# calderpg/fast_kinematic_simulator

Hardware: NVIDIA B200
Metric: particle-microsteps/sec (with contact resolution) (higher is better)
Workload: dtype f64

## Files before the change

### fast_kinematic_simulator_b200/csrc/fks_api.cu

```cuda

#include <cuda_runtime.h>
#include <nvtx3/nvToolsExt.h>

#include <algorithm>
#include <cmath>
#include <cstdio>
#include <cstdlib>
#include <cstring>
#include <new>
#include <string>
#include <vector>

#include "fks_device_types.h"
#include "fks_internal.h"

using namespace fksdev;

namespace fks_host {
static thread_local std::string g_last_error;
void set_last_error(const std::string& msg) { g_last_error = msg; }

void finish_env_l2_window(fks_env* env) {
    cudaDeviceProp prop;
    if (cudaGetDeviceProperties(&prop, env->device) == cudaSuccess && prop.persistingL2CacheMaxSize > 0) {
// ... 521 lines not shown
    s->last_stream = nullptr;
    s->has_last = false;
    {
        int lim = 0;
        if (cudaDeviceGetAttribute(&lim, cudaDevAttrMaxSharedMemoryPerBlockOptin, env->device) != cudaSuccess || lim <= 0) lim = 48 * 1024;
        s->smem_limit = (size_t)lim;
    }
    s->launches = 0;
    s->d_trace = nullptr;
    s->d_trace_count = nullptr;
    s->trace_capacity = 0;
    const double freq = std::fabs(simulation_controller_frequency);
    s->sp.interval = 1.0 / simulation_controller_frequency;
    s->sp.shortcut_distance = params->simulation_shortcut_distance;
    s->sp.check_tolerance = params->environment_collision_check_tolerance;
    s->sp.decay_rate = params->resolve_correction_step_scaling_decay_rate;
    s->sp.initial_step = params->resolve_correction_initial_step_size;
    s->sp.min_scaling = params->resolve_correction_min_step_scaling;
    s->sp.max_iters = params->max_resolver_iterations;
    s->sp.decay_iters = params->resolve_correction_step_scaling_decay_iterations;
    s->sp.n_steps = std::max((uint32_t)(params->forward_simulation_time * freq), 1u);
    s->sp.failed_ends_motion = params->failed_resolves_end_motion ? 1 : 0;

    const DevRobot& h = robot->host;
    std::memset(&s->plan, 0, sizeof(s->plan));
    int wpb = kWarpsPerBlock;
    if (const char* ev = std::getenv("FKS_WARPS_PER_BLOCK")) {
        const int v = std::atoi(ev);
        if (v >= 1 && v <= kWarpsPerBlock) wpb = v;
    }
    int rc = 0;
    for (;; wpb = (wpb > 4) ? wpb - 4 : wpb - 1) {
        s->dyn_smem = simulate_smem_plan(&s->plan, h.L, h.J, h.D, h.P, robot->stride, wpb, s->smem_limit);
        s->kinfo.max_blocks_per_sm = 0;
        rc = simulate_kernel_info(h.kind, s->dyn_smem, wpb, &s->kinfo);
        if ((rc == 0 && s->kinfo.max_blocks_per_sm >= 1) || wpb <= 1) break;
        cudaGetLastError();
    }
    s->plan.cull_mode = 1;
    s->plan.trace = nullptr;
    s->plan.trace_count = nullptr;
    s->plan.trace_capacity = 0;
    s->plan.trace_width = 0;
    if (const char* ev = std::getenv("FKS_CULL")) s->plan.cull_mode = std::atoi(ev);
    if (rc != 0) { delete s; return cuda_fail((cudaError_t)rc, "fks_sim_create: kernel attributes"); }
    if (s->kinfo.max_blocks_per_sm < 1) { delete s; return fail(FKS_ERR_UNSUPPORTED, "fks_sim_create: robot does not fit one CTA's shared memory"); }
    cudaDeviceProp prop;
    cudaError_t err = cudaGetDeviceProperties(&prop, s->device);
    if (err != cudaSuccess) { delete s; return cuda_fail(err, "cudaGetDeviceProperties"); }
    s->grid_max = prop.multiProcessorCount * s->kinfo.max_blocks_per_sm;
    s->num_sms = prop.multiProcessorCount;
    s->pool_eighths = 16;
    if (const char* ev = std::getenv("FKS_POOL_EIGHTHS")) s->pool_eighths = std::max(8, std::atoi(ev));
    s->pool = std::min((s->pool_eighths * wpb + 7) / 8, kMaxPool);
    const size_t scratch_bytes = (size_t)s->grid_max * s->pool * s->plan.sl.total;
    const size_t jscratch_bytes = (size_t)s->grid_max * wpb * s->plan.sl.jtotal;
    s->plan.pool = s->pool;
    s->plan.ctx_stride = (int)context_bytes(s->plan.wl);
    const size_t ctx_bytes = (size_t)s->grid_max * s->pool * (size_t)s->plan.ctx_stride;

    if ((err = cudaStreamCreateWithFlags(&s->stream, cudaStreamNonBlocking)) != cudaSuccess ||
        (err = cudaEventCreateWithFlags(&s->last_done, cudaEventDisableTiming)) != cudaSuccess ||
        (err = cudaMalloc((void**)&s->d_scratch, scratch_bytes)) != cudaSuccess ||
        (err = cudaMalloc((void**)&s->d_jscratch, jscratch_bytes)) != cudaSuccess ||
        (err = cudaMalloc((void**)&s->d_ctx_store, ctx_bytes)) != cudaSuccess ||
        (err = cudaMalloc((void**)&s->d_stats, 128 * sizeof(unsigned long long))) != cudaSuccess ||
        (err = cudaMalloc((void**)&s->d_counter, 4 * sizeof(unsigned int))) != cudaSuccess ||
        (err = cudaMemset(s->d_stats, 0, 128 * sizeof(unsigned long long))) != cudaSuccess) {
        fks_sim_destroy(s);
        return cuda_fail(err, "fks_sim_create: allocation");
    }
    char buf[512];
    std::snprintf(buf, sizeof(buf),
                  "simulate_kernel<kind=%d>: %d regs/thread, %zu B dynamic smem/CTA, %d B local/thread, %d threads/CTA, "
                  "%d CTAs/SM x %d SMs (persistent grid %d), scratch %llu B/warp, L2 window %zu B",
                  h.kind, s->kinfo.regs, s->dyn_smem, s->kinfo.local_bytes, 32 * wpb, s->kinfo.max_blocks_per_sm,
                  prop.multiProcessorCount, s->grid_max, (unsigned long long)s->plan.sl.jtotal, env->l2_window_bytes);
// ... 630 lines not shown
```

### fast_kinematic_simulator_b200/csrc/fks_device_types.h

```cpp
#ifndef FKS_DEVICE_TYPES_H
#define FKS_DEVICE_TYPES_H

#include <stdint.h>

#include "fksgpu.h"

namespace fksdev {

constexpr int kMaxDof = 16;
constexpr int kMaxLinks = 16;
constexpr int kMaxJoints = 16;
constexpr int kMaxPairs = (kMaxLinks * (kMaxLinks - 1)) / 2;
constexpr int kMaxSelfPartners = kMaxLinks - 1;
constexpr int kPairChunks = (kMaxPairs + 31) / 32;
#ifndef FKS_MAX_WARPS
#define FKS_MAX_WARPS 24
#endif
constexpr int kWarpsPerBlock = FKS_MAX_WARPS;
constexpr int kThreadsPerBlock = kWarpsPerBlock * 32;

struct DevAxis {
    double kp, ki, kd, iclamp;
    double vlim;
    double pnoise, mnoise;
// ... 81 lines not shown
    int M;
    int jsm;
    int jsm_ld;
    int jsm_big_ld;
    int jaxis, jorig;
    int target, scfg, act, ru, du, raw, stepv;
    int tn;
    int qr;
    int cand;
    int vars;
    int flags;
    int save2_end;
    int stats;
    int total;
    int noise_batch;
};

inline __host__ __device__ WarpLayout make_warp_layout(int L, int J, int D, int stride, int jsm_extra = 0) {
    WarpLayout w;
    int S = stride > D ? stride : D;
    S = (S + 1) & ~1;
    w.S = S;
    w.L12 = 12 * L;
    w.noise_batch = 32 / D < 1 ? 1 : (32 / D > 8 ? 8 : 32 / D);
    int o = 0;
    w.cfg = o; o += 3 * S;
    w.T = o; o += 3 * w.L12;
    w.jsm = w.T + 2 * w.L12;
    w.M = o; o += 16 * J;
    w.caps = o; o += 6 * L;
    o += jsm_extra;
    auto pick_ld = [](int doubles, int columns) {
        const int cap = doubles / columns;
        int ld = cap;
        const int pref = cap - ((cap - 4) & 15);
        if (cap >= 20 && pref >= 20 && pref * 4 >= cap * 3) ld = pref;
        return ld < 0 ? 0 : ld;
    };
    w.jsm_ld = pick_ld(o - w.jsm, D + 1);
    o += (14 + 16 - (o - w.T) % 16) % 16;
    w.G = o; o += w.L12;
    w.jaxis = o; o += 3 * J;
    w.jorig = o; o += 3 * J;
    o = (o + 1) & ~1;
    w.cand = o; o += 32;
    w.jsm_big_ld = pick_ld(o - w.jsm, D + 1);
    w.target = o; o += S;
    w.scfg = o; o += S;
    w.act = o; o += S;
    w.ru = o; o += S;
    w.du = o; o += S;
    w.raw = o; o += S;
    w.stepv = o; o += S;
    w.tn = o; o += w.noise_batch * S;
    w.vars = o; o += kWarpVarsDoubles + 2 * S;
    w.flags = o; o += 1;
    w.save2_end = o;
    w.qr = o; o += S;
    w.stats = o; o += FKS_NUM_STATS;
    w.total = (o + 1) & ~1;
    return w;
}

struct ScratchLayout {
    unsigned long long selfcorr;
    unsigned long long selfwork;
    unsigned long long keys;
// ... 52 lines not shown
    int pool, ctx_stride;
    unsigned long long n_particles, n_targets, seed, first_id;
    unsigned long long leg_id_stride;
    int n_legs;
    int allow_contacts, noise_mode, cfg_stride, rec_stride;
    int P, warps_per_block;
    int pts_off, warps_off;
    int sync_off;
    int cull_mode;
    char* trace;
    unsigned int* trace_count;
    unsigned int trace_capacity;
    int trace_width;
};

constexpr int kMaxPool = 64;

struct Frame {
    LaunchArgs a;
    DevRobot rb;
    double gbase[12];
    double pair_reach_sq[kMaxPairs];
};

struct KernelInfo {
    int regs, static_smem, local_bytes, max_blocks_per_sm;
    size_t dyn_smem;
};
int simulate_kernel_info(int kind, size_t dyn_smem, int warps_per_block, KernelInfo* out);
int launch_simulate(int kind, const LaunchArgs& args, int grid, size_t dyn_smem, void* stream,
                    const void* l2_window_base, size_t l2_window_bytes);
size_t context_bytes(const WarpLayout& wl);
constexpr size_t kSyncBytes = 16 + 2 * kMaxPool + 4 * kMaxPool;
size_t simulate_smem_plan(LaunchArgs* args, int L, int J, int D, int P, int stride, int warps_per_block, size_t smem_limit);
int launch_check_config(int kind, const LaunchArgs& args, int grid, size_t dyn_smem, void* stream, double inflation_ratio, unsigned char* out);
int launch_qr_solve(double* work, const unsigned long long* offsets, const int* rows, int cols, int n, double* x_out, unsigned* flags_out,
                    void* stream);
int launch_partition(const char* results, size_t rec_stride, int cfg_stride, size_t n, unsigned* block_counts, unsigned long long* totals,
                     unsigned* order, void* stream);
int launch_pairwise_distance(int kind, const DevRobot* robot, const char* results, size_t rec_stride, int cfg_stride, const unsigned* subset,
                             unsigned m, double* out, void* stream);
constexpr unsigned kClusterSmallMax = 160;
constexpr unsigned kClusterMaxSegment = 8192;
struct ClusterLaunch {
    const DevRobot* robot;
    const char* results;
    size_t rec_stride;
    int cfg_stride;
    int complete, separate_contact;
    double threshold;
    const unsigned* order;
    const unsigned long long* offsets;
    unsigned n_segments;
    const unsigned* small_segs;
    unsigned n_small, small_cap;
    const unsigned* large_segs;
    unsigned n_large, large_cap;
    double* work;
    int large_slots;
    unsigned* labels;
    unsigned* counts;
    unsigned long long* totals;
};
int launch_cluster(int kind, const ClusterLaunch& c, void* stream);
int launch_dbg_copy(unsigned long long* out, void* stream);
int launch_fp64_peak(double* out, int grid, int iters, void* stream);
// ... 6 lines not shown
```

### fast_kinematic_simulator_b200/csrc/fks_kernels.cu

```cuda

#include <cuda_runtime.h>
#include <float.h>
#include <math.h>
#include <stdint.h>

#include "fks_device_types.h"
#include "fks_philox.h"

namespace fksdev {

#define FKS_FULL 0xffffffffu
#ifndef FKS_SKIP_SINGLE_ESTIMATE
#define FKS_SKIP_SINGLE_ESTIMATE 1
#endif
#ifndef FKS_MIN_BLOCKS
#define FKS_MIN_BLOCKS 1
#endif

extern __shared__ __align__(16) unsigned char smem_raw[];

namespace {

constexpr double kPi = 3.14159265358979323846;

__device__ __forceinline__ const Frame& frame() { return *reinterpret_cast<const Frame*>(smem_raw); }
__device__ __forceinline__ double* wsd(int wb) { return reinterpret_cast<double*>(smem_raw + wb); }
__device__ __forceinline__ int lane_id() { return threadIdx.x & 31; }
__device__ __forceinline__ void raise_flag(int wb, unsigned bits) {
    atomicOr(reinterpret_cast<unsigned*>(wsd(wb) + frame().a.wl.flags), bits);
}
__device__ __forceinline__ void add_stat(int wb, int which, unsigned long long v) {
    reinterpret_cast<unsigned long long*>(wsd(wb) + frame().a.wl.stats)[which] += v;
}
template <class T>
__device__ __forceinline__ T wv_add(T* field, T inc) {
    const T v = *field + inc;
    __syncwarp();
    *field = v;
    return v;
}
__device__ __forceinline__ char* context_scratch(int wb) {
    const LaunchArgs& a = frame().a;
    const int ctx = reinterpret_cast<const WarpVars*>(wsd(wb) + a.wl.vars)->ctx;
    return a.scratch + ((size_t)blockIdx.x * a.pool + ctx) * a.sl.total;
}
__device__ __forceinline__ double* warp_jstore() {
    const LaunchArgs& a = frame().a;
    return reinterpret_cast<double*>(a.jscratch + ((size_t)blockIdx.x * a.warps_per_block + (threadIdx.x >> 5)) * a.sl.jtotal);
}

__device__ __noinline__ void trace_append(unsigned kind, unsigned step, unsigned micro, unsigned iter, const double* values, int n) {
    const LaunchArgs& a = frame().a;
    const int lane = lane_id();
    unsigned idx = 0u;
    if (lane == 0) idx = atomicAdd(a.trace_count, 1u);
    idx = __shfl_sync(FKS_FULL, idx, 0);
    if (idx >= a.trace_capacity) return;
    char* rec = a.trace + (size_t)idx * (sizeof(fks_trace_header) + (size_t)a.trace_width * 8);
    if (lane == 0) {
        fks_trace_header h;
        h.kind = kind;
        h.step = step;
        h.microstep = micro;
        h.iteration = iter;
        *reinterpret_cast<fks_trace_header*>(rec) = h;
    }
    double* v = reinterpret_cast<double*>(rec + sizeof(fks_trace_header));
    for (int i = lane; i < a.trace_width; i += 32) v[i] = i < n ? values[i] : 0.0;
}

__device__ __forceinline__ double warp_max(double v) {
#pragma unroll
// ... 978 lines not shown
    if (!anyc) return false;
    if (!self_pairs_share_a_cell(wb, Xcur, cp[0], cp[1], cp[2], cp[3])) return false;
    return self_collisions_exact(wb, Xprev, Xcur, cp[0], cp[1], cp[2], cp[3]);
}

#ifdef FKS_PHASE_TIMERS
__device__ unsigned long long g_dbg[64];
#endif
template <int KIND>
__device__ __forceinline__ unsigned check_collision(int wb, int Xprev, int Xcur, int use_cull) {
#ifdef FKS_PHASE_TIMERS
    const long long t0 = clock64();
#endif
    const bool envc = check_env(wb, Xcur, use_cull, 0.0);
#ifdef FKS_PHASE_TIMERS
    const long long t1 = clock64();
#endif
    const bool has_self = (KIND == FKS_ROBOT_LINKED) ? collect_self(wb, Xprev, Xcur) : false;
#ifdef FKS_PHASE_TIMERS
    if (lane_id() == 0) {
        const long long t2 = clock64();
        atomicAdd(&g_dbg[min((int)((t1 - t0) >> 11), 15)], 1ull);
        atomicAdd(&g_dbg[16 + min((int)((t2 - t1) >> 11), 15)], 1ull);
        atomicAdd(&g_dbg[32], (unsigned long long)(t1 - t0));
        atomicAdd(&g_dbg[33], (unsigned long long)(t2 - t1));
        atomicAdd(&g_dbg[34 + (envc ? 1 : 0)], 1ull);
        atomicAdd(&g_dbg[36 + (envc ? 1 : 0)], (unsigned long long)(t1 - t0));
        atomicAdd(&g_dbg[38 + (has_self ? 1 : 0)], 1ull);
    }
#endif
    return ((envc || has_self) ? 1u : 0u) | (has_self ? 2u : 0u);
}

template <int KIND>
__device__ __noinline__ int collect_corrections(int wb, int Xprev, int Xcur, bool has_self) {
    const Frame& fr = frame();
    const DevRobot& rb = fr.rb;
    const DevEnv& e = fr.a.env;
    const WarpLayout& wl = fr.a.wl;
    const int lane = lane_id();
    const int P = fr.a.P, D = rb.D;
    double* ws = wsd(wb);
    const double* Tprev = ws + wl.T + Xprev * wl.L12;
    const double* Tcur = ws + wl.T + Xcur * wl.L12;
    const double* G = ws + wl.G;
    const double2* pxy = reinterpret_cast<const double2*>(smem_raw + fr.a.pts_off);
    const PointZL* pzl = reinterpret_cast<const PointZL*>(pxy + P);
    const char* cslot = context_scratch(wb);
    double* Ag = warp_jstore();
    const unsigned char* sflag = reinterpret_cast<const unsigned char*>(cslot + fr.a.sl.sflag);
    const double* selfcorr = reinterpret_cast<const double*>(cslot + fr.a.sl.selfcorr);
    uint2* cand_s = reinterpret_cast<uint2*>(ws + wl.cand);
    uint2* cand_g = reinterpret_cast<uint2*>(Ag + (size_t)(D + 1) * fr.a.sl.ldj);
    double* jaxis = ws + wl.jaxis;
    double* jorig = ws + wl.jorig;
    if (KIND == FKS_ROBOT_LINKED) {
        for (int j = lane; j < rb.J; j += 32) {
            const DevJoint& jd = rb.joints[j];
            const double* Tj = Tcur + 12 * jd.child;
            jaxis[3 * j + 0] = Tj[0] * jd.axis[0] + Tj[1] * jd.axis[1] + Tj[2] * jd.axis[2];
            jaxis[3 * j + 1] = Tj[4] * jd.axis[0] + Tj[5] * jd.axis[1] + Tj[6] * jd.axis[2];
            jaxis[3 * j + 2] = Tj[8] * jd.axis[0] + Tj[9] * jd.axis[1] + Tj[10] * jd.axis[2];
            jorig[3 * j + 0] = Tj[3];
            jorig[3 * j + 1] = Tj[7];
            jorig[3 * j + 2] = Tj[11];
        }
// ... 114 lines not shown
                    A[0 * ld + row0 + r] = t0;
                    A[1 * ld + row0 + r] = t1;
                    A[2 * ld + row0 + r] = t2;
                    A[3 * ld + row0 + r] = t1 * (-lz) + t2 * ly;
                    A[4 * ld + row0 + r] = t0 * lz + t2 * (-lx);
                    A[5 * ld + row0 + r] = t0 * (-ly) + t1 * lx;
                }
            } else {
                const unsigned anc = rb.link_ancestors[l];
                for (int a = 0; a < D; a++) {
                    const int j = rb.active_joint[a];
                    double jx = 0.0, jy = 0.0, jz = 0.0;
                    if ((anc >> j) & 1u) {
                        const double ax = jaxis[3 * j], ay = jaxis[3 * j + 1], az = jaxis[3 * j + 2];
                        if (rb.joints[j].type == FKS_JOINT_PRISMATIC) {
                            jx = ax; jy = ay; jz = az;
                        } else {
                            const double rx = wx - jorig[3 * j], ry = wy - jorig[3 * j + 1], rz = wz - jorig[3 * j + 2];
                            jx = ay * rz - az * ry;
                            jy = az * rx - ax * rz;
                            jz = ax * ry - ay * rx;
                        }
                    }
                    double* col = A + (size_t)a * ld + row0;
                    col[0] = jx;
                    col[1] = jy;
                    col[2] = jz;
                }
            }
        }
        npts += __popc(mask);
    }
    __syncwarp();
    return 3 * npts;
}

__device__ __forceinline__ void spill_system(int wb, int cols) {
    const Frame& fr = frame();
    const WarpLayout& wl = fr.a.wl;
    const int lane = lane_id();
    const double* As = wsd(wb) + wl.jsm;
    double* Ag = warp_jstore();
    const int lds = wl.jsm_ld, cap_s = (wl.jsm_ld / 3) * 3, ldg = fr.a.sl.ldj;
    for (int c = 0; c <= cols; c++)
        for (int r = lane; r < cap_s; r += 32) Ag[(size_t)c * ldg + r] = As[c * lds + r];
    __syncwarp();
}
__device__ __forceinline__ void place_tall_system(int wb, int rows, int cols, double** store, int* store_ld) {
    const Frame& fr = frame();
    const WarpLayout& wl = fr.a.wl;
    const int lane = lane_id();
    double* As = wsd(wb) + wl.jsm;
    double* Ag = warp_jstore();
    const int ldg = fr.a.sl.ldj, ldb = wl.jsm_big_ld;
    *store = Ag;
    *store_ld = ldg;
    if (rows > ldb) return;
    for (int c = 0; c <= cols; c++)
        for (int r = lane; r < rows; r += 32) As[c * ldb + r] = __ldcg(Ag + (size_t)c * ldg + r);
    __syncwarp();
    *store = As;
    *store_ld = ldb;
}

__device__ __forceinline__ double mul_rn(double a, double b) { return __dmul_rn(a, b); }
__device__ __forceinline__ double add_rn(double a, double b) { return __dadd_rn(a, b); }
__device__ __forceinline__ double sub_rn(double a, double b) { return __dsub_rn(a, b); }
__device__ __forceinline__ double div_rn(double a, double b) { return __ddiv_rn(a, b); }
__device__ __forceinline__ double quad_sum(unsigned mask, double p) {
    p = add_rn(p, __shfl_xor_sync(mask, p, 2));
    return add_rn(p, __shfl_xor_sync(mask, p, 1));
}

#define FKS_QR_INNER_LOOP _Pragma("unroll 1")
#ifndef FKS_QR_BATCH
#define FKS_QR_BATCH 2
#endif
template <int SLOTS>
__device__ __noinline__ void colpiv_qr_lanes(int wb, double* A, int ld, int rows, int cols, int x_off) {
    const Frame& fr = frame();
    const int lane = lane_id();
    double* ws = wsd(wb);
    WarpVars* wv = reinterpret_cast<WarpVars*>(ws + fr.a.wl.vars);
    double* x = ws + x_off;
    const int g = lane >> 2, i = lane & 3;
    const unsigned quad = 0xFu << (lane & ~3);
    bool forced = false;
    int f_rank = 0;
    unsigned long long f_order = 0ull;
    if (fr.a.dec_tape != nullptr) {
        const unsigned long long dp = wv->dec_pos;
        bool desync = true, replaced = false;
        if (dp < wv->dec_end) {
            const unsigned long long* rec = fr.a.dec_tape + dp * (unsigned long long)(2 + cols);
            const unsigned long long w0 = rec[0];
// ... 268 lines not shown
    __syncwarp();
}

}

#ifndef FKS_FREE_ROUNDS
#define FKS_FREE_ROUNDS 3
#endif
#ifndef FKS_CONTACT_ROUNDS
#define FKS_CONTACT_ROUNDS(KIND) ((KIND) == FKS_ROBOT_LINKED ? 1 : 2)
#endif
#ifndef FKS_SOLVE_BATCH_EIGHTHS
#define FKS_SOLVE_BATCH_EIGHTHS 8
#endif
namespace {
enum { OP_NONE = 0, OP_KIN = 1, OP_APPLY = 2 };
enum { M_NONE = 0, M_MOTION = 1, M_CHECK = 2 };
enum {
    AF_FETCH = 0,
    AF_INIT,
    AF_EST_RU,
    AF_EST_DU,
    AF_MICRO_CHECK,
    AF_EST_RAW,
    AF_RESOLVE_CHECK,
    AF_FAIL_KIN,
    AF_STOP_KIN,
    AF_NOCONTACT_KIN,
    AF_DONE
};
enum { NEED_EMPTY = 0, NEED_ROUND = 1, NEED_SOLVE = 2, NEED_DEAD = 3 };
constexpr unsigned kLegPending = 0x80000000u;

#ifndef FKS_COPY_UNROLL
#define FKS_COPY_UNROLL 4
#endif
__device__ __forceinline__ void context_copy(double* ws, double* g, const WarpLayout& wl, bool to_global) {
    const int lane = lane_id();
    const int n0 = wl.T + 2 * wl.L12 - wl.cfg, n1 = wl.L12, n2 = wl.save2_end - wl.target;
    if (to_global) {
        for (int e = lane; e < n0; e += 32) __stcg(g + e, ws[wl.cfg + e]);
        for (int e = lane; e < n1; e += 32) __stcg(g + n0 + e, ws[wl.G + e]);
        for (int e = lane; e < n2; e += 32) __stcg(g + n0 + n1 + e, ws[wl.target + e]);
    } else {
        for (int e = lane; e < n0; e += 32) ws[wl.cfg + e] = __ldcg(g + e);
        for (int e = lane; e < n1; e += 32) ws[wl.G + e] = __ldcg(g + n0 + e);
        for (int e = lane; e < n2; e += 32) ws[wl.target + e] = __ldcg(g + n0 + n1 + e);
    }
    __syncwarp();
}
}

template <int KIND, bool TRACE = false, bool SEQ = false>
__global__ void __launch_bounds__(kThreadsPerBlock, FKS_MIN_BLOCKS) simulate_kernel(const __grid_constant__ LaunchArgs args) {
    {
        Frame* f = reinterpret_cast<Frame*>(smem_raw);
        const unsigned* src = reinterpret_cast<const unsigned*>(&args);
        unsigned* dst = reinterpret_cast<unsigned*>(&f->a);
        for (int i = threadIdx.x; i < (int)(sizeof(LaunchArgs) / 4); i += blockDim.x) dst[i] = src[i];
        const unsigned* rsrc = reinterpret_cast<const unsigned*>(args.robot);
        unsigned* rdst = reinterpret_cast<unsigned*>(&f->rb);
        for (int i = threadIdx.x; i < (int)(sizeof(DevRobot) / 4); i += blockDim.x) rdst[i] = rsrc[i];
        double2* pxy = reinterpret_cast<double2*>(smem_raw + args.pts_off);
        PointZL* pzl = reinterpret_cast<PointZL*>(pxy + args.P);
        for (int i = threadIdx.x; i < args.P; i += blockDim.x) {
            pxy[i] = args.pxy[i];
            pzl[i] = args.pzl[i];
        }
        if (threadIdx.x < 12) {
            const int r = threadIdx.x >> 2, c = threadIdx.x & 3;
            const double* io = args.env.inv_origin;
            const double* bs = args.robot->base;
            double v = io[4 * r + 0] * bs[c] + io[4 * r + 1] * bs[4 + c] + io[4 * r + 2] * bs[8 + c];
            if (c == 3) v += io[4 * r + 3];
            f->gbase[threadIdx.x] = v * args.env.inv_sdf_res;
        }
        for (int q = threadIdx.x; q < args.robot->n_pairs; q += blockDim.x) {
            const DevRobot* r = args.robot;
            const int la = r->pair_a[q], lb = r->pair_b[q];
            double ha = 0.0, hb = 0.0;
            for (int k = 0; k < 3; k++) {
                const double da = r->cap_p1[la][k] - r->cap_p0[la][k], db = r->cap_p1[lb][k] - r->cap_p0[lb][k];
                ha += da * da;
                hb += db * db;
            }
            const double diag = 2.0 * 1.7320508075688772 * args.env.map_res * (1.0 + 1e-6) + 1e-9;
            const double reach = (0.5 * sqrt(ha) + 0.5 * sqrt(hb) + r->cap_radius[la] + r->cap_radius[lb] + diag) * (1.0 + 1e-9);
            f->pair_reach_sq[q] = reach * reach;
        }
    }
    __syncthreads();
    const Frame& fr = frame();
    const LaunchArgs& a = fr.a;
    const DevRobot& rb = fr.rb;
    const WarpLayout& wl = a.wl;
    const DevSolver& sp = a.sp;
    const int lane = lane_id();
    const int warp = (int)(threadIdx.x >> 5);
    const int wb = a.warps_off + warp * wl.total * 8;
    double* ws = wsd(wb);
    const int D = rb.D, S = wl.S, stride = a.cfg_stride;
    if (lane < FKS_NUM_STATS) reinterpret_cast<unsigned long long*>(ws + wl.stats)[lane] = 0ull;
    __syncwarp();
    const double target_microstep_distance = a.env.map_res * 0.125;
    const double allowed_microstep_distance = a.env.map_res * 1.0;
    WarpVars* wv = reinterpret_cast<WarpVars*>(ws + wl.vars);
    double* pid_state = ws + wl.vars + kWarpVarsDoubles;

    const int n_warps = a.warps_per_block, pool = a.pool;
    unsigned char* need = smem_raw + a.sync_off + 16;
    signed char* holds = reinterpret_cast<signed char*>(need + kMaxPool);
    volatile unsigned* exhausted = reinterpret_cast<volatile unsigned*>(smem_raw + a.sync_off);
    char* store = a.ctx_store + (size_t)blockIdx.x * pool * a.ctx_stride;
    for (int c = threadIdx.x; c < kMaxPool; c += blockDim.x) {
        need[c] = c < n_warps ? NEED_ROUND : (c < pool ? NEED_EMPTY : NEED_DEAD);
        holds[c] = c < n_warps ? (signed char)c : (signed char)-1;
    }
    if (threadIdx.x == 0) *exhausted = 0u;
    if (lane == 0) {
        wv->after = AF_FETCH;
        wv->op = OP_NONE;
        wv->measure = M_NONE;
        wv->want_solve = 0;
        wv->cc = 0u;
        wv->cur = wv->prev = 0;
        wv->m_result = 0.0;
        wv->ctx = warp;
        if (SEQ) wv->leg = 0u;
    }
    __syncwarp();

#ifdef FKS_PHASE_TIMERS
    long long tacc[12] = {0, 0, 0, 0, 0, 0, 0, 0, 0, 0, 0, 0};
    long long tqr[4] = {0, 0, 0, 0};
    long long textra[4] = {0, 0, 0, 0};
    long long t0 = clock64(), t1;
#define FKS_TICK(i) { t1 = clock64(); tacc[i] += t1 - t0; t0 = t1; }
    long long tcyc[4] = {0, 0, 0, 0};
    long long tc_start = clock64();
    int last_kind = -1;
    __shared__ unsigned cyc_max[8];
    long long tmax[8] = {0, 0, 0, 0, 0, 0, 0, 0};
    if (threadIdx.x < 8) cyc_max[threadIdx.x] = 0u;
#define FKS_MAXTICK(i, since) { if (lane == 0) { const unsigned dt_ = (unsigned)(clock64() - (since)); atomicMax(&cyc_max[i], dt_); if ((i) == 0 || (i) == 2 || (i) == 3) atomicAdd(&g_dbg[((i) == 0 ? 40 : ((i) == 2 ? 48 : 56)) + min((int)(dt_ >> 11), 7)], 1ull); } }
#else
#define FKS_TICK(i)
#define FKS_MAXTICK(i, since)
#endif
    for (;;) {
        __syncthreads();
#ifdef FKS_PHASE_TIMERS
        {
            const long long now = clock64();
            if (last_kind >= 0) {
                tcyc[2 * last_kind] += now - tc_start;
                tcyc[2 * last_kind + 1] += 1;
            }
            tc_start = now;
            for (int i = 0; i < 8; i++) tmax[i] += cyc_max[i];
        }
        __syncthreads();
// ... 11 lines not shown
        if (ns + nr == 0 && !can_admit) break;
        const int round_supply = nr + (can_admit ? __popc(e_lo) + __popc(e_hi) : 0);
        int want = NEED_ROUND;
        if (ns > 0 && 8 * ns >= FKS_SOLVE_BATCH_EIGHTHS * n_warps) want = NEED_SOLVE;
        else if (2 * round_supply < n_warps && ns > round_supply) want = NEED_SOLVE;
        else if (round_supply == 0) want = NEED_SOLVE;
        const bool solve_phase = want != NEED_ROUND;
#ifdef FKS_PHASE_TIMERS
        last_kind = solve_phase ? 1 : 0;
#endif
        const bool keeps = h >= 0 && need[h] == want;
        const unsigned keep_mask = __ballot_sync(FKS_FULL, keeps);
        const unsigned held_lo = __reduce_or_sync(FKS_FULL, (h >= 0 && h < 32) ? (1u << h) : 0u);
        const unsigned held_hi = __reduce_or_sync(FKS_FULL, (h >= 32) ? (1u << (h - 32)) : 0u);
        const unsigned r_lo = __ballot_sync(FKS_FULL, n_lo == want) & ~held_lo, r_hi = __ballot_sync(FKS_FULL, n_hi == want) & ~held_hi;
        const int my = (int)holds[warp];
        const bool keep = (keep_mask >> warp) & 1u;
        bool active = keep;
        int got = -1;
        bool fresh = false;
        if (!keep) {
            const int rank = __popc(~keep_mask & ((1u << warp) - 1u));
            const int n_r_lo = __popc(r_lo), n_ready = n_r_lo + __popc(r_hi);
            if (rank < n_ready) {
                got = rank < n_r_lo ? (int)__fns(r_lo, 0, rank + 1) : 32 + (int)__fns(r_hi, 0, rank - n_r_lo + 1);
            } else if (!solve_phase && can_admit) {
                const int k = rank - n_ready, n_e_lo = __popc(e_lo);
                if (k < n_e_lo + __popc(e_hi)) {
                    got = k < n_e_lo ? (int)__fns(e_lo, 0, k + 1) : 32 + (int)__fns(e_hi, 0, k - n_e_lo + 1);
                    fresh = true;
                }
            }
            if (got >= 0) {
                if (my >= 0) context_copy(ws, reinterpret_cast<double*>(store + (size_t)my * a.ctx_stride), wl, true);
                if (fresh) {
                    if (lane == 0) {
                        wv->after = AF_FETCH;
                        wv->op = OP_NONE;
                        wv->measure = M_NONE;
                        wv->want_solve = 0;
                        wv->cc = 0u;
                        wv->cur = wv->prev = 0;
                        wv->m_result = 0.0;
                        wv->ctx = got;
                        if (SEQ) wv->leg = 0u;
                    }
                    __syncwarp();
                } else {
                    context_copy(ws, reinterpret_cast<double*>(store + (size_t)got * a.ctx_stride), wl, false);
                }
                if (lane == 0) holds[warp] = (signed char)got;
                active = true;
            }
        }
        const int ctx = keep ? my : got;
        FKS_MAXTICK(3, tm_swap)
        FKS_TICK(1)
        if (active) {
        int after = wv->after, op = wv->op, op_in = wv->op_in, op_out = wv->op_out, op_u = wv->op_u, op_tn = wv->op_tn,
            op_derive = wv->op_derive, measure = wv->measure, cur = wv->cur, prev = wv->prev;
        bool want_solve = wv->want_solve != 0;
        unsigned cc = wv->cc;
        double m_result = wv->m_result;
        __syncwarp();
        if (!solve_phase) {
        const int n_rounds = (ns == 0) ? 1 + FKS_FREE_ROUNDS : FKS_CONTACT_ROUNDS(KIND);
        for (int round = 0; round < n_rounds && !want_solve && after != AF_DONE; round++) {
#ifdef FKS_PHASE_TIMERS
        const long long tmA = clock64();
#endif
        if (op == OP_KIN) kinematics<KIND>(wb, op_out, op_derive);
        else if (op == OP_APPLY) apply_control<KIND>(wb, op_in, op_out, op_u, op_tn, op_derive);
        FKS_MAXTICK(0, tmA)
        FKS_TICK(0)
#ifdef FKS_PHASE_TIMERS
        const long long tmB = clock64();
#endif
        if (measure == M_MOTION) m_result = max_motion(wb, op_in, op_out);
        else if (measure == M_CHECK) cc = check_collision<KIND>(wb, prev, cur, a.cull_mode == 2 ? ((cc & 1u) ? 0 : 1) : a.cull_mode);
        FKS_MAXTICK(1, tmB)
        FKS_TICK(2)
#ifdef FKS_PHASE_TIMERS
        const long long tmT = clock64();
#endif
// ... 270 lines not shown
                }
            } else {
                ev = 0;
                if (wv->collided) wv->flags |= FKS_FLAG_DID_CONTACT;
                __syncwarp();
                wv->flags |= *reinterpret_cast<const unsigned*>(ws + wl.flags);
                char* rec = a.results + (size_t)wv->pid * a.rec_stride;
                if (SEQ) rec += (size_t)wv->leg * a.n_particles * a.rec_stride;
                if (lane < stride) reinterpret_cast<double*>(rec)[lane] = ws[wl.cfg + cur * S + lane];
                if (lane == 0) {
                    unsigned* tail = reinterpret_cast<unsigned*>(rec + (size_t)stride * 8);
                    tail[0] = wv->flags;
                    tail[1] = wv->n_micro_total;
                    tail[2] = wv->n_iter_total;
                    tail[3] = wv->n_steps;
                    add_stat(wb, FKS_STAT_TOTAL_MICROSTEPS, wv->n_micro_total);
                    add_stat(wb, FKS_STAT_TOTAL_RESOLVER_ITERATIONS, wv->n_iter_total);
                }
                __syncwarp();
                after = AF_FETCH;
                if (SEQ && wv->leg + 1u < (unsigned)a.n_legs) wv_add(&wv->leg, 1u | kLegPending);
            }
        }
        }
        FKS_MAXTICK(2, tmT)
        FKS_TICK(4)
        }
        } else {
            int rows = 0;
#ifdef FKS_PHASE_TIMERS
            const long long tc0 = clock64();
            textra[1] += 1;
#endif
            double* jstore = ws + wl.jsm;
            int jld = wl.jsm_ld;
            rows = collect_corrections<KIND>(wb, prev, cur, (cc & 2u) != 0u);
            if (lane == 0) add_stat(wb, FKS_STAT_TOTAL_CORRECTED_POINTS, (unsigned long long)(rows / 3));
            if (rows > (wl.jsm_ld / 3) * 3) {
                spill_system(wb, D);
                place_tall_system(wb, rows, D, &jstore, &jld);
            }
#ifdef FKS_PHASE_TIMERS
            tacc[10] += clock64() - tc0;
            tacc[11] += 1;
#endif
            FKS_MAXTICK(4, tc0)
            FKS_TICK(6)
            {
#ifdef FKS_PHASE_TIMERS
            const long long tq0 = clock64();
#endif
            if (rows == 0) {
                wv->flags |= FKS_FLAG_EMPTY_JACOBIAN;
                if (lane < D) ws[wl.raw + lane] = 0.0;
                __syncwarp();
            } else {
                colpiv_qr_solve(wb, jstore, jld, rows, D, wl.raw);
                __syncwarp();
            }
#ifdef FKS_PHASE_TIMERS
            if (jstore == ws + wl.jsm) { tqr[0] += clock64() - tq0; tqr[1] += 1; } else { tqr[2] += clock64() - tq0; tqr[3] += 1; }
            FKS_MAXTICK(5, tq0)
            const long long te0 = clock64();
#endif
            apply_control<KIND>(wb, cur, 2, wl.raw, -1, 0);
            m_result = max_motion(wb, cur, 2);
#ifdef FKS_PHASE_TIMERS
            textra[3] += clock64() - te0;
#endif
            FKS_MAXTICK(6, te0)
            {
                const double step_fraction = fmax(m_result / allowed_microstep_distance, 1.0);
                if (lane < D) ws[wl.stepv + lane] = (ws[wl.raw + lane] / step_fraction) * fabs(wv->scaling);
                __syncwarp();
            }
            op = OP_APPLY; op_in = cur; op_out = cur; op_u = wl.stepv; op_tn = -1; op_derive = 1;
            measure = M_CHECK;
            after = AF_RESOLVE_CHECK;
            want_solve = false;
            }
            FKS_TICK(8)
        }
        __syncwarp();
        if (lane == 0) {
            wv->after = after; wv->op = op; wv->op_in = op_in; wv->op_out = op_out; wv->op_u = op_u; wv->op_tn = op_tn;
            wv->op_derive = op_derive; wv->measure = measure; wv->cur = cur; wv->prev = prev;
            wv->want_solve = want_solve ? 1 : 0;
            wv->cc = cc;
            wv->m_result = m_result;
            need[ctx] = want_solve ? NEED_SOLVE : (after == AF_DONE ? NEED_DEAD : NEED_ROUND);
            if (after == AF_DONE) *exhausted = 1u;
        }
        __syncwarp();
        }
#ifdef FKS_PHASE_TIMERS
        textra[0] += 1;
        if (solve_phase) textra[2] += 1;
#endif
        FKS_TICK(9)
    }
#ifdef FKS_PHASE_TIMERS
    if (lane == 0)
    {
        for (int i = 0; i < 12; i++) atomicAdd(a.stats + 16 + i, (unsigned long long)tacc[i]);
        for (int i = 0; i < 4; i++) atomicAdd(a.stats + 28 + i, (unsigned long long)tqr[i]);
        for (int i = 0; i < 4; i++) atomicAdd(a.stats + 32 + i, (unsigned long long)textra[i]);
        if (warp == 0) {
            for (int i = 0; i < 4; i++) atomicAdd(a.stats + 36 + i, (unsigned long long)tcyc[i]);
            for (int i = 0; i < 8; i++) atomicAdd(a.stats + 40 + i, (unsigned long long)tmax[i]);
        }
    }
#endif
    __syncwarp();
    if (lane < FKS_NUM_STATS) {
        const unsigned long long v = reinterpret_cast<const unsigned long long*>(ws + wl.stats)[lane];
        if (v) atomicAdd(a.stats + lane, v);
    }
}

namespace {
__device__ __noinline__ bool self_collision_bool(int wb, int X, double check_resolution) {
    const Frame& fr = frame();
    const DevRobot& rb = fr.rb;
    const DevEnv& e = fr.a.env;
// ... 163 lines not shown
            x ^= x >> 7;
            x ^= x << 17;
            acc += __ldg(data + (x & n_mask));
        }
    }
    if (acc == 123.456f) out[0] = acc;
}

size_t simulate_smem_plan(LaunchArgs* args, int L, int J, int D, int P, int stride, int warps_per_block, size_t smem_limit) {
    args->sl = make_scratch_layout(D, P);
    args->P = P;
    args->warps_per_block = warps_per_block;
    const size_t pts_off = (sizeof(Frame) + 15) & ~(size_t)15;
    const size_t warps_off = pts_off + (size_t)P * (sizeof(double2) + sizeof(PointZL));
    const WarpLayout w0 = make_warp_layout(L, J, D, stride, 0);
    const size_t base = warps_off + (size_t)warps_per_block * w0.total * 8 + kSyncBytes;
    int extra = 0;
    if (smem_limit > base) {
        const long long spare = (long long)((smem_limit - base) / (size_t)warps_per_block / 8);
        int want_ld = 3 * P < 255 ? 3 * P : 255;
        want_ld |= 1;
        const long long want = (long long)(D + 1) * want_ld - (long long)(12 * L + 16 * J + 6 * L);
        long long e = want < spare ? want : spare;
        if (e < 0) e = 0;
        extra = (int)(e & ~1ll);
        while (extra > 0 && warps_off + (size_t)warps_per_block * make_warp_layout(L, J, D, stride, extra).total * 8 + kSyncBytes > smem_limit) extra -= 2;
    }
    args->wl = make_warp_layout(L, J, D, stride, extra);
    args->pts_off = (int)pts_off;
    args->warps_off = (int)warps_off;
    size_t off = warps_off + (size_t)warps_per_block * args->wl.total * 8;
    args->sync_off = (int)off;
    off += kSyncBytes;
    return off;
}

template <int KIND>
static const void* kernel_ptr_of(bool trace, bool seq) {
    if (trace) return (const void*)simulate_kernel<KIND, true>;
    return seq ? (const void*)simulate_kernel<KIND, false, true> : (const void*)simulate_kernel<KIND>;
}
static const void* kernel_ptr(int kind, bool trace = false, bool seq = false) {
    switch (kind) {
        case FKS_ROBOT_SE2: return kernel_ptr_of<FKS_ROBOT_SE2>(trace, seq);
        case FKS_ROBOT_SE3: return kernel_ptr_of<FKS_ROBOT_SE3>(trace, seq);
        case FKS_ROBOT_LINKED: return kernel_ptr_of<FKS_ROBOT_LINKED>(trace, seq);
    }
    return nullptr;
}

size_t context_bytes(const WarpLayout& wl) { return (size_t)((wl.T + 2 * wl.L12 - wl.cfg) + wl.L12 + (wl.save2_end - wl.target)) * 8; }

int simulate_kernel_info(int kind, size_t dyn_smem, int warps_per_block, KernelInfo* out) {
    const void* fn = kernel_ptr(kind);
    if (!fn) return (int)cudaErrorInvalidValue;
    cudaError_t err = cudaFuncSetAttribute(fn, cudaFuncAttributeMaxDynamicSharedMemorySize, (int)dyn_smem);
    if (err != cudaSuccess) return (int)err;
    cudaFuncAttributes fa;
    err = cudaFuncGetAttributes(&fa, fn);
    if (err != cudaSuccess) return (int)err;
    int nb = 0;
    err = cudaOccupancyMaxActiveBlocksPerMultiprocessor(&nb, fn, 32 * warps_per_block, dyn_smem);
    if (err != cudaSuccess) return (int)err;
    out->regs = fa.numRegs;
    out->static_smem = (int)fa.sharedSizeBytes;
    out->local_bytes = (int)fa.localSizeBytes;
    out->max_blocks_per_sm = nb;
    out->dyn_smem = dyn_smem;
    return 0;
}

int launch_simulate(int kind, const LaunchArgs& args, int grid, size_t dyn_smem, void* stream,
                    const void* l2_window_base, size_t l2_window_bytes) {
    const int block_threads = 32 * args.warps_per_block;
    const void* fn = kernel_ptr(kind, args.trace != nullptr, args.n_legs > 1);
    if (!fn) return (int)cudaErrorInvalidValue;
    {
        const cudaError_t err = cudaFuncSetAttribute(fn, cudaFuncAttributeMaxDynamicSharedMemorySize, (int)dyn_smem);
        if (err != cudaSuccess) return (int)err;
    }
    cudaLaunchConfig_t cfg = {};
    cfg.gridDim = dim3((unsigned)grid);
    cfg.blockDim = dim3((unsigned)block_threads);
    cfg.dynamicSmemBytes = dyn_smem;
// ... 466 lines not shown
```

Baseline: 65.05 million.

## Use TMA bulk async copies for context swaps and tall-system spill

Replaces the lane-strided global/shared copy loops used for warp context parking and reloading with cp.async.bulk stores and loads, tracked by a per-warp mbarrier in the sync area. The tall Jacobian system spill and reload now also go through bulk copies, issued inside collect_corrections. The warp layout is forced to 16-byte alignment and context strides are padded to 128 bytes. Creation now fails if the layout is not aligned. The aim is to cut per-lane load/store instruction overhead and latency on context switches, in exchange for single-lane issue, serialized waits, and extra alignment padding.

Result: faster. 67.44 million, median of 6 (+3.7%).

```diff
diff --git a/fast_kinematic_simulator_b200/csrc/fks_api.cu b/fast_kinematic_simulator_b200/csrc/fks_api.cu
--- a/fast_kinematic_simulator_b200/csrc/fks_api.cu
+++ b/fast_kinematic_simulator_b200/csrc/fks_api.cu
@@ -577,6 +577,7 @@
     int rc = 0;
     for (;; wpb = (wpb > 4) ? wpb - 4 : wpb - 1) {
         s->dyn_smem = simulate_smem_plan(&s->plan, h.L, h.J, h.D, h.P, robot->stride, wpb, s->smem_limit);
+        if (s->dyn_smem == 0) break;
         s->kinfo.max_blocks_per_sm = 0;
         rc = simulate_kernel_info(h.kind, s->dyn_smem, wpb, &s->kinfo);
         if ((rc == 0 && s->kinfo.max_blocks_per_sm >= 1) || wpb <= 1) break;
@@ -588,6 +589,7 @@
     s->plan.trace_capacity = 0;
     s->plan.trace_width = 0;
     if (const char* ev = std::getenv("FKS_CULL")) s->plan.cull_mode = std::atoi(ev);
+    if (s->dyn_smem == 0) { delete s; return fail(FKS_ERR_UNSUPPORTED, "fks_sim_create: warp block layout not 16-byte aligned for bulk copies"); }
     if (rc != 0) { delete s; return cuda_fail((cudaError_t)rc, "fks_sim_create: kernel attributes"); }
     if (s->kinfo.max_blocks_per_sm < 1) { delete s; return fail(FKS_ERR_UNSUPPORTED, "fks_sim_create: robot does not fit one CTA's shared memory"); }
     cudaDeviceProp prop;
diff --git a/fast_kinematic_simulator_b200/csrc/fks_device_types.h b/fast_kinematic_simulator_b200/csrc/fks_device_types.h
--- a/fast_kinematic_simulator_b200/csrc/fks_device_types.h
+++ b/fast_kinematic_simulator_b200/csrc/fks_device_types.h
@@ -137,7 +137,7 @@
     o += jsm_extra;
     auto pick_ld = [](int doubles, int columns) {
         const int cap = doubles / columns;
-        int ld = cap;
+        int ld = cap & ~1;
         const int pref = cap - ((cap - 4) & 15);
         if (cap >= 20 && pref >= 20 && pref * 4 >= cap * 3) ld = pref;
         return ld < 0 ? 0 : ld;
@@ -256,6 +256,8 @@
                     const void* l2_window_base, size_t l2_window_bytes);
 size_t context_bytes(const WarpLayout& wl);
 constexpr size_t kSyncBytes = 16 + 2 * kMaxPool + 4 * kMaxPool;
+constexpr size_t kSyncBarOff = 16 + 2 * kMaxPool;
+static_assert(kSyncBarOff % 8 == 0 && kSyncBarOff + 8 * kWarpsPerBlock <= kSyncBytes, "one mbarrier per warp in the sync area");
 size_t simulate_smem_plan(LaunchArgs* args, int L, int J, int D, int P, int stride, int warps_per_block, size_t smem_limit);
 int launch_check_config(int kind, const LaunchArgs& args, int grid, size_t dyn_smem, void* stream, double inflation_ratio, unsigned char* out);
 int launch_qr_solve(double* work, const unsigned long long* offsets, const int* rows, int cols, int n, double* x_out, unsigned* flags_out,
diff --git a/fast_kinematic_simulator_b200/csrc/fks_kernels.cu b/fast_kinematic_simulator_b200/csrc/fks_kernels.cu
--- a/fast_kinematic_simulator_b200/csrc/fks_kernels.cu
+++ b/fast_kinematic_simulator_b200/csrc/fks_kernels.cu
@@ -38,6 +38,37 @@
     __syncwarp();
     *field = v;
     return v;
+}
+
+__device__ __forceinline__ unsigned smem_u32(const void* p) { return (unsigned)__cvta_generic_to_shared(p); }
+__device__ __forceinline__ void fence_async_shared() { asm volatile("fence.proxy.async.shared::cta;" ::: "memory"); }
+__device__ __forceinline__ void fence_async_global() { asm volatile("fence.proxy.async.global;" ::: "memory"); }
+__device__ __forceinline__ void bulk_store(double* g, const double* s, int doubles) {
+    asm volatile("cp.async.bulk.global.shared::cta.bulk_group [%0], [%1], %2;" ::"l"(g), "r"(smem_u32(s)), "r"(doubles * 8)
+                 : "memory");
+}
+__device__ __forceinline__ void bulk_commit() { asm volatile("cp.async.bulk.commit_group;" ::: "memory"); }
+__device__ __forceinline__ void bulk_wait_read() { asm volatile("cp.async.bulk.wait_group.read 0;" ::: "memory"); }
+__device__ __forceinline__ void bulk_wait_all() { asm volatile("cp.async.bulk.wait_group 0;" ::: "memory"); }
+__device__ __forceinline__ unsigned warp_bar() {
+    return smem_u32(smem_raw + frame().a.sync_off + kSyncBarOff) + 8u * (threadIdx.x >> 5);
+}
+__device__ __forceinline__ unsigned long long bulk_expect(unsigned bar, int bytes) {
+    unsigned long long state;
+    asm volatile("mbarrier.arrive.expect_tx.shared::cta.b64 %0, [%1], %2;" : "=l"(state) : "r"(bar), "r"(bytes) : "memory");
+    return state;
+}
+__device__ __forceinline__ void bulk_load(double* s, const double* g, int doubles, unsigned bar) {
+    asm volatile("cp.async.bulk.shared::cluster.global.mbarrier::complete_tx::bytes [%0], [%1], %2, [%3];"
+                 ::"r"(smem_u32(s)), "l"(g), "r"(doubles * 8), "r"(bar) : "memory");
+}
+__device__ __forceinline__ void bulk_wait_loads(unsigned bar, unsigned long long state) {
+    state = __shfl_sync(FKS_FULL, state, 0);
+    unsigned done;
+    do {
+        asm volatile("{ .reg .pred p; mbarrier.try_wait.shared::cta.b64 p, [%1], %2; selp.u32 %0, 1, 0, p; }"
+                     : "=r"(done) : "r"(bar), "l"(state) : "memory");
+    } while (!done);
 }
 __device__ __forceinline__ char* context_scratch(int wb) {
     const LaunchArgs& a = frame().a;
@@ -1082,6 +1113,36 @@
     return ((envc || has_self) ? 1u : 0u) | (has_self ? 2u : 0u);
 }
 
+__device__ __forceinline__ void move_tall_system(int wb, int rows, int cols) {
+    const Frame& fr = frame();
+    const WarpLayout& wl = fr.a.wl;
+    const int lane = lane_id();
+    double* As = wsd(wb) + wl.jsm;
+    double* Ag = warp_jstore();
+    const int lds = wl.jsm_ld, cap_s = (wl.jsm_ld / 3) * 3, ldg = fr.a.sl.ldj, ldb = wl.jsm_big_ld;
+    const int nb = cap_s & ~1;
+    if (nb < cap_s && lane <= cols) Ag[(size_t)lane * ldg + nb] = As[lane * lds + nb];
+    fence_async_shared();
+    fence_async_global();
+    __syncwarp();
+    if (lane == 0) {
+        for (int c = 0; c <= cols; c++) bulk_store(Ag + (size_t)c * ldg, As + c * lds, nb);
+        bulk_commit();
+        bulk_wait_all();
+    }
+    __syncwarp();
+    if (rows > ldb) return;
+    const int n = (rows + 1) & ~1;
+    const unsigned bar = warp_bar();
+    unsigned long long state = 0ull;
+    if (lane == 0) {
+        fence_async_global();
+        state = bulk_expect(bar, (cols + 1) * n * 8);
+        for (int c = 0; c <= cols; c++) bulk_load(As + c * ldb, Ag + (size_t)c * ldg, n, bar);
+    }
+    bulk_wait_loads(bar, state);
+}
+
 template <int KIND>
 __device__ __noinline__ int collect_corrections(int wb, int Xprev, int Xcur, bool has_self) {
     const Frame& fr = frame();
@@ -1262,35 +1323,8 @@
         npts += __popc(mask);
     }
     __syncwarp();
+    if (3 * npts > cap_s) move_tall_system(wb, 3 * npts, D);
     return 3 * npts;
-}
-
-__device__ __forceinline__ void spill_system(int wb, int cols) {
-    const Frame& fr = frame();
-    const WarpLayout& wl = fr.a.wl;
-    const int lane = lane_id();
-    const double* As = wsd(wb) + wl.jsm;
-    double* Ag = warp_jstore();
-    const int lds = wl.jsm_ld, cap_s = (wl.jsm_ld / 3) * 3, ldg = fr.a.sl.ldj;
-    for (int c = 0; c <= cols; c++)
-        for (int r = lane; r < cap_s; r += 32) Ag[(size_t)c * ldg + r] = As[c * lds + r];
-    __syncwarp();
-}
-__device__ __forceinline__ void place_tall_system(int wb, int rows, int cols, double** store, int* store_ld) {
-    const Frame& fr = frame();
-    const WarpLayout& wl = fr.a.wl;
-    const int lane = lane_id();
-    double* As = wsd(wb) + wl.jsm;
-    double* Ag = warp_jstore();
-    const int ldg = fr.a.sl.ldj, ldb = wl.jsm_big_ld;
-    *store = Ag;
-    *store_ld = ldg;
-    if (rows > ldb) return;
-    for (int c = 0; c <= cols; c++)
-        for (int r = lane; r < rows; r += 32) As[c * ldb + r] = __ldcg(Ag + (size_t)c * ldg + r);
-    __syncwarp();
-    *store = As;
-    *store_ld = ldb;
 }
 
 __device__ __forceinline__ double mul_rn(double a, double b) { return __dmul_rn(a, b); }
@@ -1625,22 +1659,34 @@
 enum { NEED_EMPTY = 0, NEED_ROUND = 1, NEED_SOLVE = 2, NEED_DEAD = 3 };
 constexpr unsigned kLegPending = 0x80000000u;
 
-#ifndef FKS_COPY_UNROLL
-#define FKS_COPY_UNROLL 4
-#endif
-__device__ __forceinline__ void context_copy(double* ws, double* g, const WarpLayout& wl, bool to_global) {
-    const int lane = lane_id();
-    const int n0 = wl.T + 2 * wl.L12 - wl.cfg, n1 = wl.L12, n2 = wl.save2_end - wl.target;
-    if (to_global) {
-        for (int e = lane; e < n0; e += 32) __stcg(g + e, ws[wl.cfg + e]);
-        for (int e = lane; e < n1; e += 32) __stcg(g + n0 + e, ws[wl.G + e]);
-        for (int e = lane; e < n2; e += 32) __stcg(g + n0 + n1 + e, ws[wl.target + e]);
-    } else {
-        for (int e = lane; e < n0; e += 32) ws[wl.cfg + e] = __ldcg(g + e);
-        for (int e = lane; e < n1; e += 32) ws[wl.G + e] = __ldcg(g + n0 + e);
-        for (int e = lane; e < n2; e += 32) ws[wl.target + e] = __ldcg(g + n0 + n1 + e);
-    }
+__device__ __forceinline__ void context_swap(double* ws, int park_ctx, int load_ctx, const WarpLayout& wl) {
+    const LaunchArgs& a = frame().a;
+    char* store = a.ctx_store + (size_t)blockIdx.x * a.pool * a.ctx_stride;
+    double* park = reinterpret_cast<double*>(store + (size_t)park_ctx * a.ctx_stride);
+    const double* load = reinterpret_cast<const double*>(store + (size_t)load_ctx * a.ctx_stride);
+    const int n0 = wl.T + 2 * wl.L12 - wl.cfg, n1 = wl.L12, n2 = (wl.save2_end - wl.target + 1) & ~1;
+    const unsigned bar = warp_bar();
+    fence_async_shared();
     __syncwarp();
+    unsigned long long state = 0ull;
+    if (lane_id() == 0) {
+        if (park_ctx >= 0) {
+            bulk_store(park, ws + wl.cfg, n0);
+            bulk_store(park + n0, ws + wl.G, n1);
+            bulk_store(park + n0 + n1, ws + wl.target, n2);
+            bulk_commit();
+            bulk_wait_read();
+        }
+        if (load_ctx >= 0) {
+            fence_async_global();
+            state = bulk_expect(bar, (n0 + n1 + n2) * 8);
+            bulk_load(ws + wl.cfg, load, n0, bar);
+            bulk_load(ws + wl.G, load + n0, n1, bar);
+            bulk_load(ws + wl.target, load + n0 + n1, n2, bar);
+        }
+    }
+    __syncwarp();
+    if (load_ctx >= 0) bulk_wait_loads(bar, state);
 }
 }
 
@@ -1704,7 +1750,6 @@
     unsigned char* need = smem_raw + a.sync_off + 16;
     signed char* holds = reinterpret_cast<signed char*>(need + kMaxPool);
     volatile unsigned* exhausted = reinterpret_cast<volatile unsigned*>(smem_raw + a.sync_off);
-    char* store = a.ctx_store + (size_t)blockIdx.x * pool * a.ctx_stride;
     for (int c = threadIdx.x; c < kMaxPool; c += blockDim.x) {
         need[c] = c < n_warps ? NEED_ROUND : (c < pool ? NEED_EMPTY : NEED_DEAD);
         holds[c] = c < n_warps ? (signed char)c : (signed char)-1;
@@ -1720,6 +1765,8 @@
         wv->m_result = 0.0;
         wv->ctx = warp;
         if (SEQ) wv->leg = 0u;
+        asm volatile("mbarrier.init.shared::cta.b64 [%0], 1;" ::"r"(warp_bar()) : "memory");
+        asm volatile("fence.mbarrier_init.release.cluster;" ::: "memory");
     }
     __syncwarp();
 
@@ -1797,7 +1844,7 @@
                 }
             }
             if (got >= 0) {
-                if (my >= 0) context_copy(ws, reinterpret_cast<double*>(store + (size_t)my * a.ctx_stride), wl, true);
+                context_swap(ws, my, fresh ? -1 : got, wl);
                 if (fresh) {
                     if (lane == 0) {
                         wv->after = AF_FETCH;
@@ -1811,10 +1858,7 @@
                         if (SEQ) wv->leg = 0u;
                     }
                     __syncwarp();
-                } else {
-                    context_copy(ws, reinterpret_cast<double*>(store + (size_t)got * a.ctx_stride), wl, false);
-                }
-                if (lane == 0) holds[warp] = (signed char)got;
+                }
                 active = true;
             }
         }
@@ -2151,13 +2195,16 @@
             const long long tc0 = clock64();
             textra[1] += 1;
 #endif
+            rows = collect_corrections<KIND>(wb, prev, cur, (cc & 2u) != 0u);
+            if (lane == 0) add_stat(wb, FKS_STAT_TOTAL_CORRECTED_POINTS, (unsigned long long)(rows / 3));
             double* jstore = ws + wl.jsm;
             int jld = wl.jsm_ld;
-            rows = collect_corrections<KIND>(wb, prev, cur, (cc & 2u) != 0u);
-            if (lane == 0) add_stat(wb, FKS_STAT_TOTAL_CORRECTED_POINTS, (unsigned long long)(rows / 3));
             if (rows > (wl.jsm_ld / 3) * 3) {
-                spill_system(wb, D);
-                place_tall_system(wb, rows, D, &jstore, &jld);
+                jld = wl.jsm_big_ld;
+                if (rows > jld) {
+                    jstore = warp_jstore();
+                    jld = a.sl.ldj;
+                }
             }
 #ifdef FKS_PHASE_TIMERS
             tacc[10] += clock64() - tc0;
@@ -2207,8 +2254,10 @@
             wv->want_solve = want_solve ? 1 : 0;
             wv->cc = cc;
             wv->m_result = m_result;
+            holds[warp] = (signed char)ctx;
             need[ctx] = want_solve ? NEED_SOLVE : (after == AF_DONE ? NEED_DEAD : NEED_ROUND);
             if (after == AF_DONE) *exhausted = 1u;
+            bulk_wait_all();
         }
         __syncwarp();
         }
@@ -2438,7 +2487,12 @@
     size_t off = warps_off + (size_t)warps_per_block * args->wl.total * 8;
     args->sync_off = (int)off;
     off += kSyncBytes;
-    return off;
+    const WarpLayout& w = args->wl;
+    const int ranges[] = {w.total, w.cfg, w.T + 2 * w.L12 - w.cfg, w.G, w.L12, w.target, w.jsm, w.jsm_ld, w.jsm_big_ld,
+                          args->sl.ldj};
+    bool aligned = warps_off % 16 == 0 && (w.save2_end + 1) / 2 * 2 <= w.total;
+    for (int v : ranges) aligned = aligned && v % 2 == 0;
+    return aligned ? off : 0;
 }
 
 template <int KIND>
@@ -2455,7 +2509,10 @@
     return nullptr;
 }
 
-size_t context_bytes(const WarpLayout& wl) { return (size_t)((wl.T + 2 * wl.L12 - wl.cfg) + wl.L12 + (wl.save2_end - wl.target)) * 8; }
+size_t context_bytes(const WarpLayout& wl) {
+    const size_t bytes = (size_t)((wl.T + 2 * wl.L12 - wl.cfg) + wl.L12 + ((wl.save2_end - wl.target + 1) & ~1)) * 8;
+    return (bytes + 127) & ~(size_t)127;
+}
 
 int simulate_kernel_info(int kind, size_t dyn_smem, int warps_per_block, KernelInfo* out) {
     const void* fn = kernel_ptr(kind);
```
